# SandraLouise/SVJedi-graph

Hardware: NVIDIA B200
Metric: gaf_alignments_filtered_assigned_per_sec (higher is better)
Workload: dtype u8/int64

## Files before the change

### svjedi-graph_b200/csrc/filter.cu

```cuda
#include <cooperative_groups.h>
#include <cuda_runtime.h>

#include <algorithm>
#include <cstdlib>
#include <map>
#include <mutex>

#include "svjg_internal.h"

namespace cg = cooperative_groups;
using namespace svjg;

namespace {

constexpr int TILE_MIN = 1024;
constexpr int TILE_LINES = 30;
constexpr int LOOKAHEAD = 1024;
constexpr int HEAD = 32;
constexpr int WARPS = 4;
constexpr int THREADS = WARPS * 32;
constexpr int SPARE = 32;

template <int MB_, int TILE_MAX_>
struct Geo {
// ... 606 lines not shown
                }
                const uint32_t idB = node_id(tok_hash(B), B);
                const int sB = strand(B);
                if (err) return;
                link(A, idA, sA, B, idB, sB, false, false);
                if (err) return;
                idA = idB;
                sA = sB;
                have_a = true;
            } else {
                have_a = false;
            }
            A = B;
        }
    }
};

__device__ __forceinline__ uint32_t smem_u32(const void *p) { return (uint32_t)__cvta_generic_to_shared(p); }
__device__ __forceinline__ void mbar_init(uint64_t *bar, uint32_t count) {
    asm volatile("mbarrier.init.shared::cta.b64 [%0], %1;" ::"r"(smem_u32(bar)), "r"(count));
    asm volatile("fence.mbarrier_init.release.cluster;" ::: "memory");
}
__device__ __forceinline__ void mbar_expect_tx(uint64_t *bar, uint32_t bytes) {
    asm volatile("mbarrier.arrive.expect_tx.shared::cta.b64 _, [%0], %1;" ::"r"(smem_u32(bar)), "r"(bytes) : "memory");
}
__device__ __forceinline__ void bulk_g2s(void *dst, const void *src, uint32_t bytes, uint64_t *bar) {
    uint64_t once;
    asm volatile("createpolicy.fractional.L2::evict_first.b64 %0, 1.0;" : "=l"(once));
    asm volatile("cp.async.bulk.shared::cluster.global.mbarrier::complete_tx::bytes.L2::cache_hint [%0], [%1], %2, [%3], %4;" ::"r"(
                     smem_u32(dst)),
                 "l"(src), "r"(bytes), "r"(smem_u32(bar)), "l"(once)
                 : "memory");
}
__device__ __forceinline__ void mbar_wait(uint64_t *bar, uint32_t parity) {
    asm volatile(
        "{\n\t.reg .pred p;\n\t"
        "WAIT_%=:\n\t"
        "mbarrier.try_wait.parity.shared::cta.b64 p, [%0], %1;\n\t"
        "@p bra DONE_%=;\n\t"
        "bra WAIT_%=;\n\t"
        "DONE_%=:\n\t}" ::"r"(smem_u32(bar)),
        "r"(parity)
        : "memory");
}

__device__ __forceinline__ void l2_prefetch(const void *src, uint32_t bytes) {
    asm volatile("cp.async.bulk.prefetch.L2.global [%0], %1;" ::"l"(src), "r"(bytes) : "memory");
}

__device__ __forceinline__ uint32_t lds32(const uint8_t *win, uint32_t a) { return *reinterpret_cast<const uint32_t *>(win + a); }

__device__ __forceinline__ bool has_comma(const uint8_t *win, uint32_t lo, uint32_t hi) {
    const uint32_t a0 = lo & ~3u, a1 = (hi - 1u) & ~3u;
    const uint32_t lom = 0xFFFFFFFFu << (8u * (lo & 3u)), him = 0xFFFFFFFFu >> (8u * (3u - ((hi - 1u) & 3u)));
    uint32_t f = eq_bytes(lds32(win, a0), 0x2C2C2C2Cu) & lom;
    if (a0 == a1) return (f & him) != 0;
    for (uint32_t a = a0 + 4; a < a1; a += 4) f |= eq_bytes(lds32(win, a), 0x2C2C2C2Cu);
    return (f | (eq_bytes(lds32(win, a1), 0x2C2C2C2Cu) & him)) != 0;
}

__device__ __forceinline__ uint32_t warp_incl_scan(uint32_t v, int lane) {
#pragma unroll
    for (int d = 1; d < 32; d <<= 1) {
        uint32_t o = __shfl_up_sync(0xFFFFFFFFu, v, d);
        if (lane >= d) v += o;
    }
    return v;
}

__device__ __forceinline__ uint64_t warp_incl_scan64(uint64_t v, int lane) {
#pragma unroll
    for (int d = 1; d < 32; d <<= 1) {
        uint64_t o = __shfl_up_sync(0xFFFFFFFFu, v, d);
        if (lane >= d) v += o;
    }
    return v;
}

__device__ __forceinline__ uint32_t bm_bits(const uint32_t *bm, uint32_t pos) {
    const uint32_t w = pos >> 5;
    return __funnelshift_r(bm[w], bm[w + 1], pos & 31u);
}
__device__ __forceinline__ uint32_t low_bits(int n) { return __funnelshift_lc(0xFFFFFFFFu, 0u, uint32_t(max(n, 0))); }
__device__ __forceinline__ uint32_t next_tab(const uint32_t *bm, uint32_t pos, uint32_t end) {
    for (uint32_t q = pos; q < end; q += 32) {
        const uint32_t m = bm_bits(bm, q) & low_bits(int(end - q));
        if (m) return q + uint32_t(__ffs(m) - 1);
    }
    return end;
}
__device__ __forceinline__ uint64_t bm64(const uint32_t *bm, uint32_t pos) {
    const uint32_t w = pos >> 5, sh = pos & 31u;
    const uint32_t b0 = bm[w], b1 = bm[w + 1], b2 = bm[w + 2];
    return (uint64_t(__funnelshift_r(b1, b2, sh)) << 32) | __funnelshift_r(b0, b1, sh);
}
__device__ __forceinline__ uint64_t low_bits64(int n) { return (uint64_t(low_bits(n - 32)) << 32) | low_bits(n); }

__device__ __forceinline__ uint32_t dec4(uint32_t w) {
    uint32_t t = w & 0x0F0F0F0Fu;
    t = t * 10u + (t >> 8);
    t &= 0x00FF00FFu;
    return (t * 100u + (t >> 16)) & 0xFFFFu;
}
__device__ __forceinline__ uint32_t clear_low_bytes(uint32_t w, int n) {
    return w & __funnelshift_lc(0u, 0xFFFFFFFFu, uint32_t(max(n, 0)) * 8u);
}
__device__ __forceinline__ bool pnode_find(const DevTables &tb, uint64_t c0, uint64_t c1, uint32_t ka, uint32_t kb,
                                           uint32_t &id, uint32_t &alt_len, uint32_t &roles) {
    uint32_t i = pnode_hash(c0, c1, ka, kb) & tb.pnode_mask;
    for (;;) {
        const uint4 *sp = reinterpret_cast<const uint4 *>(tb.pnodes + i);
        const uint4 lo = __ldg(sp), hi = __ldg(sp + 1);
        if (!hi.z) return false;
        if (lo.x == uint32_t(c0) && lo.y == uint32_t(c0 >> 32) && lo.z == uint32_t(c1) && lo.w == uint32_t(c1 >> 32) &&
            hi.x == ka && hi.y == kb) {
            id = (hi.z & PN_ID_MASK) - 1u;
            roles = hi.z >> 28;
            alt_len = hi.w;
            return true;
        }
        i = (i + 1) & tb.pnode_mask;
    }
}

__device__ __forceinline__ uint32_t link_dirs(uint32_t rolesA, uint32_t sA, uint32_t rolesB, uint32_t sB) {
    const uint32_t fwd = (rolesA >> sA) & (rolesB >> (2u + sB)) & 1u;
    const uint32_t rev = (rolesB >> (sB ^ 1u)) & (rolesA >> (2u + (sA ^ 1u))) & 1u;
    return fwd | (rev << 1);
}

struct SmemBytes {
    const uint8_t *p;
    __device__ __forceinline__ uint32_t u8(uint32_t i) const { return p[i]; }
    __device__ __forceinline__ uint32_t u32(uint32_t al) const { return *reinterpret_cast<const uint32_t *>(p + al); }
};
struct ShardBytes {
    const FilterArgs *a;
    __device__ __forceinline__ uint32_t u8(uint32_t i) const { return i < a->n ? __ldg(a->gaf + i) : 0u; }
    __device__ __forceinline__ uint32_t u32(uint32_t al) const { return gaf_word(*a, al); }
};

template <class B>
__device__ __forceinline__ uint32_t dec9(const B &src, uint32_t hi, uint32_t n) {
    const uint32_t base = hi - 8u, al = base & ~3u, sh = (base & 3u) * 8u;
    const uint32_t r0 = src.u32(al), r1 = src.u32(al + 4), r2 = src.u32(al + 8);
    const int m = 8 - int(min(n, 8u));
    const uint32_t g0 = dec4(clear_low_bytes(__funnelshift_r(r0, r1, sh), m));
    const uint32_t g1 = dec4(clear_low_bytes(__funnelshift_r(r1, r2, sh), m - 4));
    uint32_t v = g0 * 10000u + g1;
    if (n == 9u) v += (src.u8(hi - 9u) - '0') * 100000000u;
    return v;
}

struct Node {
    uint32_t nid = NO_NODE;
    uint32_t nlen = 0;
    uint32_t akey = 0;
    uint32_t roles = 0;
    bool plain = false;
};
template <class B>
__device__ __forceinline__ Node resolve_node(const B &src, const uint32_t *xdb, const DevTables &tb, uint32_t tpos, uint32_t tend) {
    Node n;
    const uint32_t L = tend - tpos;
    const uint32_t Y = bm_bits(xdb, tend - 32u) | low_bits(32 - int(L));
    const uint32_t n2 = uint32_t(__clz(int(Y)));
    const uint32_t n1 = uint32_t(__clz(int(Y << ((n2 + 1u) & 31u))));
    const int clen = int(L) - int(n1 + n2 + 2u);
    if (n2 - 1u <= 8u && n1 - 1u <= 8u && uint32_t(clen) <= 15u) {
        const uint32_t q2 = tend - n2, sep = q2 - 1u, q1 = sep - n1, col = q1 - 1u;
        const uint32_t cs = src.u8(sep);
        bool ok = (cs == '-' || cs == '.') && src.u8(col) == ':';
        ok = ok && !(n1 > 1u && src.u8(q1) == '0') && !(n2 > 1u && src.u8(q2) == '0');
        const uint32_t al = tpos & ~3u, sh = (tpos & 3u) * 8u;
        const uint32_t r0 = src.u32(al), r1 = src.u32(al + 4), r2 = src.u32(al + 8), r3 = src.u32(al + 12), r4 = src.u32(al + 16);
        const uint32_t w0 = __funnelshift_r(r0, r1, sh) & low_bits(8 * clen);
        const uint32_t w1 = __funnelshift_r(r1, r2, sh) & low_bits(8 * clen - 32);
        const uint32_t w2 = __funnelshift_r(r2, r3, sh) & low_bits(8 * clen - 64);
        const uint32_t w3 = (__funnelshift_r(r3, r4, sh) & low_bits(8 * clen - 96)) | (uint32_t(clen) << 24);
        auto has_colon = [](uint32_t w) {
            const uint32_t x = w ^ 0x3A3A3A3Au;
            return (x - 0x01010101u) & ~x & SVJG_H8;
        };
        ok = ok && (has_colon(w0) | has_colon(w1) | has_colon(w2) | has_colon(w3 & 0x00FFFFFFu)) == 0u;
        if (ok) {
            const uint32_t v0 = dec9(src, sep, n1), v1 = dec9(src, tend, n2);
            const uint32_t kind = cs == '.' ? PN_ALT : 0u;
            uint32_t id = NO_NODE, alt_len = PN_NO_LEN;
            const bool found = pnode_find(tb, (uint64_t(w1) << 32) | w0, (uint64_t(w3) << 32) | w2, v0, v1 | kind, id, alt_len, n.roles);
            n.akey = v0 | kind;
            if (!kind) {
                if (v1 >= v0) {
                    n.plain = true;
                    n.nlen = v1 - v0 + 1u;
                    n.nid = found ? id : NO_NODE;
                }
            } else if (found && alt_len != PN_NO_LEN) {
                n.plain = true;
                n.nlen = alt_len;
                n.nid = id;
            }
        }
    }
    return n;
}

__device__ __forceinline__ uint32_t find_node(const uint32_t *nsb, uint32_t lps, uint32_t idx) {
    uint32_t w = lps >> 5, rem = idx;
    uint32_t bits = nsb[w] & ~low_bits(int(lps & 31u));
    for (;;) {
        const uint32_t c = __popc(bits);
        if (rem < c) break;
        rem -= c;
        bits = nsb[++w];
    }
    for (; rem; --rem) bits &= bits - 1;
    return w * 32u + uint32_t(__ffs(bits) - 1);
}
__device__ __forceinline__ uint32_t next_node(const uint32_t *nsb, uint32_t pos, uint32_t end) { return next_tab(nsb, pos, end); }

__device__ __forceinline__ void probe_links(const FilterArgs &a, bool want, uint32_t idl, uint32_t sl, uint32_t idr, uint32_t sr,
                                            uint32_t dirs, bool ok, uint32_t off, uint32_t len, uint32_t lt_mask, uint32_t &n_checks) {
#pragma unroll 1
    for (uint32_t pass = 0; pass < 2; ++pass) {
        const bool act = want && (pass ? dirs == 3u : dirs != 0u);
        if (pass && !__any_sync(0xFFFFFFFFu, act)) break;
        const bool fwd = pass == 0 && (dirs & 1u);
        const uint32_t kl = fwd ? idl : idr, kr = fwd ? idr : idl, ksl = fwd ? sl : sr ^ 1u, ksr = fwd ? sr : sl ^ 1u;
        const uint32_t key_lo = (kr << 1) | ksr, key_hi = (kl << 1) | ksl;
        uint4 sv = make_uint4(0, 0, 0, 0);
        uint32_t i = link_hash((uint64_t(key_hi) << 32) | key_lo);
        bool go = act, match = false;
        while (__any_sync(0xFFFFFFFFu, go)) {
            if (go) {
                i &= a.tb.link_mask;
                sv = __ldg(reinterpret_cast<const uint4 *>(a.tb.links + i));
                match = (sv.w & 1u) && sv.x == key_lo && sv.y == key_hi;
                go = (sv.w & 1u) && !match;
                ++i;
            }
        }
        const bool poisoned = match && (sv.w & 8u);
        const uint32_t cnt = (match && !poisoned) ? sv.w >> 4 : 0u;
        n_checks += cnt;
        const uint32_t mine = ok ? cnt : 0u;
        uint32_t before, total;
        if (__any_sync(0xFFFFFFFFu, mine > 1u)) {
            const uint32_t incl = warp_incl_scan(mine, int(threadIdx.x & 31));
            before = incl - mine;
            total = __shfl_sync(0xFFFFFFFFu, incl, 31);
        } else {
            const uint32_t hb = __ballot_sync(0xFFFFFFFFu, mine != 0u);
            before = __popc(hb & lt_mask);
            total = __popc(hb);
        }
        if (total) {
            unsigned long long base = 0;
            if ((threadIdx.x & 31) == 0) base = atomicAdd(a.stats + 0, (unsigned long long)total);
            base = __shfl_sync(0xFFFFFFFFu, base, 0) + before;
            for (uint32_t k = 0; k < mine; ++k) {
                const uint32_t sv2 = cnt == 1u ? sv.z : __ldg(a.tb.entries + sv.z + k);
                if (sv2 == ENTRY_POISON) {
                    report(a, SVJG_BAD_ENTRY, off);
                    break;
                }
                atomicAdd(a.counts + sv2, 1u);
                if (base + k < a.hit_cap) {
                    __stcs(a.hit_sv2 + base + k, sv2);
                    if (a.hit_off64) __stcs(reinterpret_cast<unsigned long long *>(a.hit_off64) + base + k, (unsigned long long)(a.base + off));
                    else __stcs(a.hit_off + base + k, off);
                    __stcs(a.hit_len + base + k, len);
                }
            }
        }
        if (poisoned) report(a, SVJG_BAD_ENTRY, off);
    }
}

constexpr int SLAB_N = 256;

template <class B>
__device__ __noinline__ bool long_line(const FilterArgs &a, const B src, const uint32_t *nsb, const uint32_t *xdb, uint4 *slab,
                                       uint32_t slab_cap, int lane, uint32_t cnt, uint32_t lps, uint32_t lpe, int64_t lts,
                                       int64_t ltail, uint32_t off, uint32_t len) {
    if (cnt > slab_cap) return false;
    const uint32_t lt_mask = (1u << lane) - 1u;
    uint32_t n_checks = 0;
    uint64_t total = 0;
    bool bad = false;
    uint32_t from = lps;
    for (uint32_t c0 = 0; c0 < cnt; c0 += 32) {
        const bool act = c0 + uint32_t(lane) < cnt;
        Node n;
        uint32_t tpos = lpe, plus = 0;
        if (act) tpos = find_node(nsb, from, uint32_t(lane));
        uint32_t nxt = __shfl_down_sync(0xFFFFFFFFu, tpos, 1);
        if (lane == 31 && act && c0 + 32u < cnt) nxt = next_node(nsb, tpos + 1u, lpe);
        if (act) {
            const uint32_t tend = c0 + uint32_t(lane) + 1u < cnt ? nxt - 1u : lpe;
            plus = src.u8(tpos - 1u) == '>';
            n = resolve_node(src, xdb, a.tb, tpos, tend);
            __stcg(slab + c0 + lane, make_uint4(n.nid, n.nlen, n.akey, plus | (n.roles << 1)));
        }
        bad |= __any_sync(0xFFFFFFFFu, act && !n.plain);
        total += __shfl_sync(0xFFFFFFFFu, warp_incl_scan64(n.nlen, lane), 31);
        from = __shfl_sync(0xFFFFFFFFu, nxt, 31);
    }
    __syncwarp();
    if (bad) return false;
    bool clash = false;
    for (uint32_t c0 = 0; c0 < cnt; c0 += 32) {
        const uint32_t t = c0 + uint32_t(lane);
        const uint32_t mine = t < cnt ? __ldcg(&slab[t].z) : 0u;
        const uint32_t upto = min(c0 + 32u, cnt);
        for (uint32_t j = 0; j < upto; ++j) clash |= j < t && t < cnt && __ldcg(&slab[j].z) == mine;
    }
    if (__any_sync(0xFFFFFFFFu, clash)) return false;
    uint64_t before = 0;
    for (uint32_t c0 = 0; c0 < cnt; c0 += 32) {
        const uint32_t t = c0 + uint32_t(lane);
        const bool act = t < cnt;
        const uint4 me = act ? __ldcg(slab + t) : make_uint4(NO_NODE, 0, 0, 0);
        const uint4 lf = act && t ? __ldcg(slab + t - 1) : make_uint4(NO_NODE, 0, 0, 0);
        const uint64_t incl = warp_incl_scan64(me.y, lane);
        const uint64_t pre = before + incl - me.y;
        const bool ok = (int64_t(pre) - lts >= a.d_over) && (int64_t(total - pre) - ltail >= a.d_over);
        const uint32_t dirs = link_dirs(lf.w >> 1, lf.w & 1u, me.w >> 1, me.w & 1u);
        const bool want = act && t && lf.x != NO_NODE && me.x != NO_NODE && dirs && (ok || (a.flags & FLAG_EXACT_CHECKS));
        probe_links(a, want, lf.x, lf.w & 1u, me.x, me.w & 1u, dirs, ok, off, len, lt_mask, n_checks);
        before += __shfl_sync(0xFFFFFFFFu, incl, 31);
    }
    n_checks = __reduce_add_sync(0xFFFFFFFFu, n_checks);
    if (lane == 0 && n_checks) atomicAdd(a.stats + 3, (unsigned long long)n_checks);
    return true;
}

template <class G>
__global__ void __launch_bounds__(THREADS, G::MB) scan_kernel(const __grid_constant__ FilterArgs a) {
    extern __shared__ __align__(128) uint8_t smem_all[];
    __shared__ __align__(8) uint64_t mbars[WARPS];
    __shared__ uint32_t next_tile[WARPS];

    const int lane = threadIdx.x & 31, warp = threadIdx.x >> 5;
    const uint32_t lt_mask = (1u << lane) - 1u;
    uint8_t *win = smem_all + warp * G::WARP_SMEM;
    uint16_t *nl = reinterpret_cast<uint16_t *>(win + G::OFF_NL);
    uint32_t *tabb = reinterpret_cast<uint32_t *>(win + G::OFF_TAB);
    uint32_t *xdb = reinterpret_cast<uint32_t *>(win + G::OFF_XD);
    uint32_t *nsb = reinterpret_cast<uint32_t *>(win + G::OFF_NS);
    uint8_t *tko = win + G::OFF_TKO;
    uint2 *lrec = reinterpret_cast<uint2 *>(win + G::OFF_LREC);
    uint64_t *mbar = &mbars[warp];
    const SmemBytes src{win};

    if (lane == 0) mbar_init(mbar, 1);
    for (int i = lane; i < G::BMWORDS; i += 32) tabb[i] = 0, xdb[i] = 0, nsb[i] = 0;
    for (int i = G::WIN + lane; i < G::WIN + SPARE; i += 32) win[i] = 0;
    __syncwarp();
    uint32_t phase = 0;
    uint32_t u_rec = 0, u_multi = 0, n_checks = 0;
    const uint32_t one = a.one;
    const uint32_t n_workers = gridDim.x * WARPS;

    cudaGridDependencySynchronize();
    cudaTriggerProgrammaticLaunchCompletion();
    const uint32_t tile_bytes = a.sc.cnt[4];
    const uint32_t n_tiles = uint32_t((a.n + tile_bytes - 1) / tile_bytes);
    const uint32_t win_bytes = HEAD + tile_bytes + LOOKAHEAD, n_pairs = win_bytes / 32u;

    for (uint32_t tile = blockIdx.x * WARPS + warp; tile < n_tiles; tile = next_tile[warp], __syncwarp()) {
        const uint64_t tile_start = uint64_t(tile) * tile_bytes;
        const uint64_t g0 = tile_start ? tile_start - HEAD : 0;
        const uint32_t dst0 = tile_start ? 0 : HEAD;
        uint64_t g1 = tile_start + tile_bytes + LOOKAHEAD;
        if (g1 > a.n) g1 = a.n;
        const bool at_eof = (g1 == a.n);
        const uint32_t nbytes = uint32_t(g1 - g0);
        const uint32_t bulk = nbytes & ~15u;
        const uint32_t valid_end = dst0 + nbytes;
        const uint32_t wbase = uint32_t(tile_start) - HEAD;

        if (lane == 0) {
            if (bulk) {
                asm volatile("fence.proxy.async.shared::cta;" ::: "memory");
                mbar_expect_tx(mbar, bulk);
                bulk_g2s(win + dst0, a.gaf + g0, bulk, mbar);
            }
            const uint32_t next = n_workers + atomicAdd(a.sc.cnt + 6, 1u);
            next_tile[warp] = next;
            const uint64_t nx = uint64_t(next) * tile_bytes;
            if (nx + tile_bytes + LOOKAHEAD <= a.n) l2_prefetch(a.gaf + nx - HEAD, win_bytes);
        }
        if (bulk != nbytes || dst0 || valid_end < win_bytes) {
            for (uint32_t i = bulk + lane; i < nbytes; i += 32) win[dst0 + i] = __ldg(a.gaf + g0 + i);
            if (dst0) win[lane] = (lane == HEAD - 1 && a.skip == 0u) ? '\n' : 0;
            for (uint32_t i = valid_end + lane; i < win_bytes; i += 32) win[i] = 0;
        }
        if (bulk) {
            mbar_wait(mbar, phase);
            phase ^= 1;
        }
        __syncwarp();

        const uint32_t own_end = min(HEAD + tile_bytes, valid_end);
        uint32_t n_nl = 0, n_own = 0;
        for (uint32_t c0 = 0; c0 < n_pairs; c0 += 32) {
            const uint32_t c = c0 + uint32_t(lane);
            const uint32_t p0 = c * 32u;
            uint32_t m = 0;
            if (c < n_pairs) {
                const uint4 v0 = *reinterpret_cast<const uint4 *>(win + p0);
                const uint4 v1 = *reinterpret_cast<const uint4 *>(win + p0 + 16);
                m = mask32(v0, v1, IsNewline{one});
                tabb[c] = mask32(v0, v1, IsTab{one});
                xdb[c] = mask32(v0, v1, IsNonDigit{one});
                const uint32_t d = mask32(v0, v1, IsDelim{one});
                const uint32_t left = c ? uint32_t(is_delim(win[p0 - 1u])) : 0u;
                nsb[c] = ((d << 1) | left) & ~d;
                if (c == 0) m &= 0x80000000u;
            }
            if (__any_sync(0xFFFFFFFFu, (m & (m - 1u)) != 0u)) {
                const uint32_t cnt = __popc(m), incl = warp_incl_scan(cnt, lane);
                uint32_t idx = n_nl + incl - cnt, own = 0;
                for (uint32_t mm = m; mm; mm &= mm - 1) {
                    const uint32_t pos = p0 + uint32_t(__ffs(mm) - 1);
                    if (idx < uint32_t(G::NLCAP)) nl[idx] = uint16_t(pos);
                    own += pos + 1u < own_end;
                    ++idx;
                }
                n_nl += __shfl_sync(0xFFFFFFFFu, incl, 31);
                n_own += __reduce_add_sync(0xFFFFFFFFu, own);
            } else {
                const uint32_t pos = p0 + uint32_t(__ffs(m)) - 1u;
                const uint32_t b = __ballot_sync(0xFFFFFFFFu, m != 0u);
                const uint32_t bo = __ballot_sync(0xFFFFFFFFu, m != 0u && pos + 1u < own_end);
                const uint32_t idx = n_nl + __popc(b & lt_mask);
                if (m != 0u && idx < uint32_t(G::NLCAP)) nl[idx] = uint16_t(pos);
                n_nl += __popc(b);
                n_own += __popc(bo);
            }
            if ((c0 + 32u) * 32u >= own_end && __any_sync(0xFFFFFFFFu, (m & ~low_bits(int(own_end) - 1 - int(p0))) != 0)) break;
        }
        __syncwarp();
        if (a.flags & FLAG_STOP_AFTER_SCAN) continue;

        if (n_nl > uint32_t(G::NLCAP)) {
            if (lane == 0) report(a, SVJG_BAD_SHORTLINE, tile_start);
            __syncwarp();
            continue;
        }
        u_rec += n_own;
        for (uint32_t k0 = 0; k0 < n_own; k0 += 32) {
            const uint32_t k = k0 + lane;
            uint32_t want = 0;
            bool exact = false;
            uint32_t s = 0, e = 0, ps = 0, pe = 0;
            uint32_t c6 = 0, c7 = 0, c8 = 0, c9 = 0;
            bool has_nl = false;
            if (k < n_own) {
                s = uint32_t(nl[k]) + 1u;
                if (k + 1 < n_nl) {
                    e = nl[k + 1];
                    has_nl = true;
                } else if (at_eof) {
                    e = valid_end;
                } else {
                    exact = true;
                }
                if (!exact) {
                    bool plain = e > s && !py_space(win[e - 1]);
                    uint32_t t1;
                    {
                        const uint64_t t64 = bm64(tabb, s) & low_bits64(int(e - s));
                        t1 = t64 ? s + uint32_t(__ffsll((long long)t64)) - 1u : next_tab(tabb, min(s + 64u, e), e);
                    }
                    plain &= t1 < e;
                    const uint32_t n2 = t1 + 1u;
                    const uint32_t tw = bm_bits(tabb, n2);
                    const uint32_t xa = bm_bits(xdb, n2) & ~tw;
                    plain &= xa != 0;
                    const uint32_t l2 = uint32_t(__ffs(xa)) - 1u;
                    const uint32_t ta = tw & low_bits(int(l2));
                    plain &= __popc(ta) == 3 && (ta >> ((l2 - 1u) & 31u)) == 1u && (ta & ((ta >> 1) | 1u)) == 0;
                    const uint32_t n5 = n2 + l2;
                    ps = (l2 < 31u && ((tw >> (l2 + 1u)) & 1u)) ? n5 + 2u : next_tab(tabb, min(n5, e), e) + 1u;
                    uint32_t ntok = 0;
                    pe = e;
                    for (uint32_t q = ps; q < e; q += 32) {
                        const uint32_t tb = bm_bits(tabb, q) & low_bits(int(e - q));
                        const uint32_t nb = bm_bits(nsb, q);
                        if (tb) {
                            const uint32_t r = uint32_t(__ffs(tb)) - 1u;
                            pe = q + r;
                            ntok += __popc(nb & low_bits(int(r)));
                            break;
                        }
                        ntok += __popc(nb);
                    }
                    plain &= pe < e && pe > ps;
                    const uint32_t n7 = min(pe + 1u, e);
                    uint64_t tt = bm64(tabb, n7);
                    const uint64_t xt = bm64(xdb, n7) & ~tt;
                    plain &= xt != 0;
                    const uint32_t l7 = uint32_t(__ffsll((long long)xt)) - 1u;
                    tt &= low_bits64(int(l7));
                    const uint32_t ntab = uint32_t(__popcll(tt));
                    const bool last_is_tab = l7 != 0 && ((tt >> ((l7 - 1u) & 63u)) & 1ull) != 0;
                    plain &= (ntab == 6 && last_is_tab) || (ntab == 5 && !last_is_tab && n7 + l7 == e);
                    plain &= (tt & ((tt >> 1) | 1ull)) == 0;
                    c6 = pe;
                    c7 = n7 + uint32_t(__ffsll((long long)tt)) - 1u;
                    tt &= tt - 1;
                    c8 = n7 + uint32_t(__ffsll((long long)tt)) - 1u;
                    tt &= tt - 1;
                    c9 = n7 + uint32_t(__ffsll((long long)tt)) - 1u;
                    tt &= tt - 1;
                    const uint32_t p10 = n7 + uint32_t(__ffsll((long long)tt)) - 1u;
                    plain = plain && win[p10 + 1] != '0';
                    if (!plain) {
                        exact = true;
                    } else if (!is_delim(win[ps])) {
                        exact = has_comma(win, ps, pe);
                    } else if (ntok >= 2) {
                        if (a.flags & FLAG_FORCE_GENERAL) exact = true;
                        else want = ntok;
                    }
                }
            }
            __syncwarp();
            int32_t ts = 0, tail = 0;
            if (want) {
                const uint32_t n_tlen = c7 - c6 - 1u, n_ts = c8 - c7 - 1u, n_te = c9 - c8 - 1u;
                if (max(n_tlen, max(n_ts, n_te)) <= 9u) {
                    ts = int32_t(dec9(src, c8, n_ts));
                    tail = int32_t(dec9(src, c7, n_tlen)) - int32_t(dec9(src, c9, n_te)) - 1;
                    lrec[lane] = make_uint2(s | ((e - s + (has_nl ? 1u : 0u)) << 16), ps | (pe << 16));
                } else {
                    exact = true;
                    want = 0;
                }
            }
            __syncwarp();
            uint32_t pend = want > 32u ? 0u : want;
            while (__any_sync(0xFFFFFFFFu, pend != 0)) {
                const uint32_t incl = warp_incl_scan(pend, lane);
                const bool take = pend != 0 && incl <= 32u;
                const uint32_t takeb = __ballot_sync(0xFFFFFFFFu, take);
                const uint32_t ntk = __shfl_sync(0xFFFFFFFFu, incl, 31 - __clz(takeb));
                const uint32_t first = incl - pend;
                const uint32_t startmask = __reduce_or_sync(0xFFFFFFFFu, take ? (1u << first) : 0u);
                if (take) tko[__popc(takeb & lt_mask)] = uint8_t(lane);
                __syncwarp();
                const bool is_tok = uint32_t(lane) < ntk;
                uint32_t own_l = 0, idx = 0;
                if (is_tok) {
                    const uint32_t below = startmask & (0xFFFFFFFFu >> (31 - lane));
                    own_l = tko[__popc(below) - 1];
                    idx = uint32_t(lane) - uint32_t(31 - __clz(below));
                }
                const uint2 lr = lrec[own_l];
                const uint32_t lpath = lr.y;
                const uint32_t lcnt = __shfl_sync(0xFFFFFFFFu, pend, own_l);
                uint32_t tpos = 0;
                if (is_tok) tpos = find_node(nsb, lpath & 0xFFFFu, idx);
                const uint32_t nxt = __shfl_down_sync(0xFFFFFFFFu, tpos, 1);
                Node nd;
                uint32_t plus = 0;
                if (is_tok) {
                    plus = win[tpos - 1u] == '>';
                    nd = resolve_node(src, xdb, a.tb, tpos, idx + 1u < lcnt ? nxt - 1u : lpath >> 16);
                }
                const uint32_t nid = nd.nid, nlen = nd.nlen, akey = nd.akey;
                const uint32_t lfirst = uint32_t(lane) - idx;
                const uint32_t line_lanes = low_bits(int(lcnt)) << lfirst;
                const uint32_t twins = __match_any_sync(0xFFFFFFFFu, akey) & line_lanes;
                bool clash = (twins & ~(1u << lane)) != 0;
                uint64_t lsum = nlen;
#pragma unroll
                for (int d = 1; d < 32; d <<= 1) {
                    const uint64_t o = __shfl_up_sync(0xFFFFFFFFu, lsum, d);
                    if (uint32_t(d) <= idx) lsum += o;
                }
                uint64_t pre_l = lsum - nlen, pre_r = pre_l;
                uint32_t splus = plus, sl = __shfl_up_sync(0xFFFFFFFFu, plus, 1);
                if (__any_sync(0xFFFFFFFFu, is_tok && clash)) {
                    const int twin0 = is_tok ? __ffs(twins) - 1 : lane;
                    const uint32_t f_nid = __shfl_sync(0xFFFFFFFFu, nid, twin0);
                    const uint64_t f_sum = __shfl_sync(0xFFFFFFFFu, lsum, twin0);
                    const uint32_t f_len = __shfl_sync(0xFFFFFFFFu, nlen, twin0);
                    splus = __shfl_sync(0xFFFFFFFFu, plus, twin0);
                    sl = __shfl_up_sync(0xFFFFFFFFu, splus, 1);
                    pre_l = __shfl_up_sync(0xFFFFFFFFu, f_sum, 1);
                    pre_r = f_sum - f_len;
                    clash = clash && !(nid != NO_NODE && f_nid == nid);
                }
                const uint32_t bad = __reduce_or_sync(0xFFFFFFFFu, (is_tok && (!nd.plain || clash)) ? (1u << own_l) : 0u);
                const uint64_t total = __shfl_sync(0xFFFFFFFFu, lsum, is_tok ? lfirst + lcnt - 1u : 0u);
                const uint32_t idl = __shfl_up_sync(0xFFFFFFFFu, nid, 1);
                const int64_t lts = __shfl_sync(0xFFFFFFFFu, ts, own_l), ltail = __shfl_sync(0xFFFFFFFFu, tail, own_l);
                const uint32_t loff = wbase + (lr.x & 0xFFFFu), llen = lr.x >> 16;
                const bool ok = (int64_t(pre_l) - lts >= a.d_over) && (int64_t(total - pre_r) - ltail >= a.d_over);
                const uint32_t dirs = link_dirs(__shfl_up_sync(0xFFFFFFFFu, nd.roles, 1), sl, nd.roles, splus);
                const bool look = is_tok && idx >= 1 && !((bad >> own_l) & 1u) && idl != NO_NODE && nid != NO_NODE && dirs &&
                                  (ok || (a.flags & FLAG_EXACT_CHECKS));
                probe_links(a, look, idl, sl, nid, splus, dirs, ok, loff, llen, lt_mask, n_checks);
                if (take) {
                    if ((bad >> lane) & 1u) exact = true;
                    pend = 0;
                }
                u_multi += __popc(takeb & ~bad);
                __syncwarp();
            }
            for (uint32_t longb = __ballot_sync(0xFFFFFFFFu, want > 32u); longb; longb &= longb - 1) {
                const int L = __ffs(longb) - 1;
                const uint2 lr = lrec[L];
                const bool done = long_line(a, src, nsb, xdb, a.sc.slab + size_t(blockIdx.x * WARPS + warp) * SLAB_N, SLAB_N, lane,
                                            __shfl_sync(0xFFFFFFFFu, want, L), lr.y & 0xFFFFu, lr.y >> 16,
                                            __shfl_sync(0xFFFFFFFFu, ts, L), __shfl_sync(0xFFFFFFFFu, tail, L),
                                            wbase + (lr.x & 0xFFFFu), lr.x >> 16);
                if (!done && lane == L) exact = true;
                u_multi += done;
            }
            const uint32_t xb = __ballot_sync(0xFFFFFFFFu, exact);
            if (xb) {
                uint32_t xbase = 0;
                if (lane == 0) xbase = atomicAdd(a.sc.cnt + 2, uint32_t(__popc(xb)));
                xbase = __shfl_sync(0xFFFFFFFFu, xbase, 0);
                if (exact) {
                    const uint32_t idx = xbase + __popc(xb & lt_mask);
                    if (idx < a.sc.cap_exact) a.sc.exact[idx] = wbase + s;
                    else report(a, SVJG_BAD_SHORTLINE, wbase + s);
                }
            }
        }
        __syncwarp();
    }
    n_checks = __reduce_add_sync(0xFFFFFFFFu, n_checks);
    if (lane == 0) {
        if (u_rec) atomicAdd(a.stats + 1, (unsigned long long)u_rec);
        if (u_multi) atomicAdd(a.stats + 2, (unsigned long long)u_multi);
        if (n_checks) atomicAdd(a.stats + 3, (unsigned long long)n_checks);
    }
}

__device__ __noinline__ bool giant_line(const FilterArgs &a, uint32_t ps, uint32_t pe, uint32_t ntok, int64_t ts, int64_t tail,
                                        uint32_t off, uint32_t len, int lane, Local &loc) {
    if (ps < 64u) return false;
    const uint32_t w0 = (ps >> 5) - 1u, nw = (pe >> 5) - w0 + 4u;
    const uint32_t bm16 = (nw + 3u) / 4u;
    const uint32_t need = 2u * bm16 + ntok;
    uint32_t base = 0;
    if (lane == 0) base = atomicAdd(a.sc.cnt + 5, need);
    base = __shfl_sync(0xFFFFFFFFu, base, 0);
    if (uint64_t(base) + need > a.sc.cap_pool) return false;
    uint32_t *nsb = reinterpret_cast<uint32_t *>(a.sc.pool + base), *xdb = reinterpret_cast<uint32_t *>(a.sc.pool + base + bm16);
    for (uint32_t w = uint32_t(lane); w < nw; w += 32) {
        const uint64_t pos = uint64_t(w0 + w) * 32u;
        uint32_t d = 0, x = 0;
        if (pos + 32 <= a.n) {
            const uint4 v0 = __ldg(reinterpret_cast<const uint4 *>(a.gaf + pos)), v1 = __ldg(reinterpret_cast<const uint4 *>(a.gaf + pos + 16));
            d = mask16(v0, IsDelim{1u}) | (mask16(v1, IsDelim{1u}) << 16);
            x = mask16(v0, IsNonDigit{1u}) | (mask16(v1, IsNonDigit{1u}) << 16);
        } else {
            for (uint32_t k = 0; k < 32; ++k) {
                const uint32_t c = pos + k < a.n ? uint32_t(__ldg(a.gaf + pos + k)) : 0u;
                d |= uint32_t(is_delim(c)) << k;
                x |= uint32_t(c - '0' > 9u) << k;
            }
        }
        const uint32_t left = uint32_t(is_delim(__ldg(a.gaf + pos - 1)));
        __stcg(nsb + w, ((d << 1) | left) & ~d);
        __stcg(xdb + w, x);
    }
    __syncwarp();
    return long_line(a, ShardBytes{&a}, nsb - w0, xdb - w0, a.sc.pool + base + 2u * bm16, ntok, lane, ntok, ps, pe, ts, tail, off, len);
}

__global__ void __launch_bounds__(FLAT_THREADS) exact_kernel(const __grid_constant__ FilterArgs a) {
    cudaGridDependencySynchronize();
    cudaTriggerProgrammaticLaunchCompletion();
    const uint32_t n = min(a.sc.cnt[2], a.sc.cap_exact);
    if (n == 0) return;
    Local loc;
    const uint32_t n_warps = gridDim.x * (FLAT_THREADS / 32);
    const bool per_warp = n <= 4u * n_warps;
    const uint32_t me = per_warp ? (blockIdx.x * FLAT_THREADS + threadIdx.x) >> 5 : blockIdx.x * FLAT_THREADS + threadIdx.x;
    const uint32_t stride = per_warp ? n_warps : gridDim.x * FLAT_THREADS;
    const uint32_t part = per_warp ? (threadIdx.x & 31u) : 0u, parts = per_warp ? 32u : 1u;
    if (blockIdx.x == 0 && threadIdx.x == 0 && n) atomicAdd(a.stats + 7, (unsigned long long)n);
    for (uint32_t i = me; i < n; i += stride) {
        const uint32_t off = a.sc.exact[i];
        uint64_t e = off;
        if (per_warp) e = coop_find(a, off, a.n, EqByte{0x0A0A0A0Au});
        else
            while (e < a.n && __ldg(a.gaf + e) != '\n') ++e;
        const uint32_t len = uint32_t(e - off) + (e < a.n ? 1u : 0u);
        Rec<GmemSrc> rec(a, GmemSrc{a.gaf}, off, len, loc);
        rec.coop = per_warp;
        const uint32_t ntok = rec.parse_fields(uint64_t(off), e);
        if (!rec.err && ntok >= 2) {
            if (ntok != COMMA_PATH && part == 0) loc.n_multi++;
            const bool fast = per_warp && ntok != COMMA_PATH && !(a.flags & FLAG_FORCE_GENERAL) && e < 0xFFFFFFFFull &&
                              giant_line(a, uint32_t(rec.ps), uint32_t(rec.pe), ntok, rec.ts, rec.tlen - rec.te - 1, off, len,
                                         int(threadIdx.x & 31u), loc);
            if (!fast) rec.general(part, parts);
        }
        if (rec.err) report(a, rec.err, off);
    }
    add_stats(a, loc);
}

constexpr int PROBE_THREADS = 1024, PROBE_BYTES = 64 << 10;

__global__ void __launch_bounds__(PROBE_THREADS) probe_kernel(const __grid_constant__ FilterArgs a) {
    cudaTriggerProgrammaticLaunchCompletion();
    __shared__ uint32_t total;
    if (threadIdx.x == 0) total = 0;
    if (threadIdx.x < 16 && threadIdx.x != 4) a.sc.cnt[threadIdx.x] = 0;
    __syncthreads();
    const uint64_t span = a.n < uint64_t(PROBE_BYTES) ? a.n : uint64_t(PROBE_BYTES);
    const uint32_t n16 = uint32_t(span / 16);
    const uint4 *p = reinterpret_cast<const uint4 *>(a.gaf);
    uint32_t cnt = 0;
    for (uint32_t i = threadIdx.x; i < n16; i += PROBE_THREADS) {
        const uint4 v = __ldg(p + i);
        cnt += __popc(eq_bytes(v.x, 0x0A0A0A0Au)) + __popc(eq_bytes(v.y, 0x0A0A0A0Au)) + __popc(eq_bytes(v.z, 0x0A0A0A0Au)) +
               __popc(eq_bytes(v.w, 0x0A0A0A0Au));
    }
    cnt = __reduce_add_sync(0xFFFFFFFFu, cnt);
    if ((threadIdx.x & 31) == 0 && cnt) atomicAdd(&total, cnt);
    __syncthreads();
    if (threadIdx.x == 0) {
        const uint32_t tile_max = a.tile_max;
        uint32_t tile = tile_max;
        if (total) {
            const uint64_t want = uint64_t(n16) * 16ull * a.tile_lines / total;
            tile = uint32_t(want < uint64_t(tile_max) ? want : uint64_t(tile_max)) & ~31u;
        }
        if (const uint32_t forced = (a.flags >> 16)) tile = forced & ~31u;
        if (total) {
            const uint64_t s15 = uint64_t(n16) * 24ull / total;
            const uint32_t slack = uint32_t(s15 < 512 ? s15 : 512);
            tile = min(tile, tile_max);
            const uint32_t steps = (HEAD + tile + slack) / 1024u;
            if (steps >= 2) tile = (steps * 1024u - HEAD - slack) & ~31u;
        }
        a.sc.cnt[4] = max(uint32_t(TILE_MIN), min(tile, tile_max));
    }
}

__global__ void reset_kernel(uint32_t *counts, uint64_t n, unsigned long long *stats) {
    uint64_t i = blockIdx.x * uint64_t(blockDim.x) + threadIdx.x;
    uint64_t stride = uint64_t(gridDim.x) * blockDim.x;
    for (uint64_t k = i; k < n; k += stride) counts[k] = 0;
    if (i < 8) stats[i] = (i == 5) ? ~0ull : 0ull;
}

template <typename... P, typename... A>
cudaError_t launch_pdl(void (*kernel)(P...), unsigned grid, unsigned block, size_t smem, cudaStream_t st, A &&...args) {
    cudaLaunchAttribute attr[1];
    attr[0].id = cudaLaunchAttributeProgrammaticStreamSerialization;
    attr[0].val.programmaticStreamSerializationAllowed = 1;
    cudaLaunchConfig_t cfg = {};
    cfg.gridDim = dim3(grid);
    cfg.blockDim = dim3(block);
    cfg.dynamicSmemBytes = smem;
    cfg.stream = st;
    cfg.attrs = attr;
    cfg.numAttrs = 1;
    return cudaLaunchKernelEx(&cfg, kernel, static_cast<A &&>(args)...);
}

struct DevCfg {
    int sms = 0;
    int grid_cap = 0;
    int min_blocks = 0;
    uint32_t tile_max = 0, tile_lines = 0;
    uint32_t smem = 0;
    cudaEvent_t ev0 = nullptr, ev1 = nullptr;
    bool timed = false;
};
std::mutex g_cfg_mu;
std::map<int, DevCfg> g_cfg;
bool g_profile = false;

struct Knobs {
    int tile_bytes = 0, tile_lines = 0, scan_blocks = 0, scan_only = 0, pool_units = 0;
};
Knobs g_knobs;

// ... 164 lines not shown
```

Measured before the change: 8.061 billion.

## Prefetch next tile's window during final node-table lookups of current tile

Splits node resolution into key parsing from the shared-memory window and a separate hash-table lookup. On the last batch of a tile, once every remaining read of the window is done, lane 0 starts the bulk async copy of the next tile's window before the table lookups run. This is meant to hide the global-to-shared copy latency behind those lookups. It also packs two per-lane counters into one register. It adds a shared flag and a condition on when the window is dead, which risks a race if any later code still reads the window.

```diff
diff --git a/svjedi-graph_b200/csrc/filter.cu b/svjedi-graph_b200/csrc/filter.cu
--- a/svjedi-graph_b200/csrc/filter.cu
+++ b/svjedi-graph_b200/csrc/filter.cu
@@ -782,6 +782,11 @@
     return v;
 }
 
+struct NodeKey {
+    uint32_t w0 = 0, w1 = 0, w2 = 0, w3 = 0;
+    uint32_t ka = 0, kb = 0;
+    bool ok = false;
+};
 struct Node {
     uint32_t nid = NO_NODE;
     uint32_t nlen = 0;
@@ -790,8 +795,8 @@
     bool plain = false;
 };
 template <class B>
-__device__ __forceinline__ Node resolve_node(const B &src, const uint32_t *xdb, const DevTables &tb, uint32_t tpos, uint32_t tend) {
-    Node n;
+__device__ __forceinline__ NodeKey node_key(const B &src, const uint32_t *xdb, uint32_t tpos, uint32_t tend) {
+    NodeKey k;
     const uint32_t L = tend - tpos;
     const uint32_t Y = bm_bits(xdb, tend - 32u) | low_bits(32 - int(L));
     const uint32_t n2 = uint32_t(__clz(int(Y)));
@@ -814,22 +819,31 @@
         };
         ok = ok && (has_colon(w0) | has_colon(w1) | has_colon(w2) | has_colon(w3 & 0x00FFFFFFu)) == 0u;
         if (ok) {
-            const uint32_t v0 = dec9(src, sep, n1), v1 = dec9(src, tend, n2);
-            const uint32_t kind = cs == '.' ? PN_ALT : 0u;
-            uint32_t id = NO_NODE, alt_len = PN_NO_LEN;
-            const bool found = pnode_find(tb, (uint64_t(w1) << 32) | w0, (uint64_t(w3) << 32) | w2, v0, v1 | kind, id, alt_len, n.roles);
-            n.akey = v0 | kind;
-            if (!kind) {
-                if (v1 >= v0) {
-                    n.plain = true;
-                    n.nlen = v1 - v0 + 1u;
-                    n.nid = found ? id : NO_NODE;
-                }
-            } else if (found && alt_len != PN_NO_LEN) {
+            k.w0 = w0, k.w1 = w1, k.w2 = w2, k.w3 = w3;
+            k.ka = dec9(src, sep, n1);
+            k.kb = dec9(src, tend, n2) | (cs == '.' ? PN_ALT : 0u);
+            k.ok = true;
+        }
+    }
+    return k;
+}
+__device__ __forceinline__ Node node_find(const DevTables &tb, const NodeKey &k) {
+    Node n;
+    if (k.ok) {
+        const uint32_t v0 = k.ka, kind = k.kb & PN_ALT, v1 = k.kb & ~PN_ALT;
+        uint32_t id = NO_NODE, alt_len = PN_NO_LEN;
+        const bool found = pnode_find(tb, (uint64_t(k.w1) << 32) | k.w0, (uint64_t(k.w3) << 32) | k.w2, k.ka, k.kb, id, alt_len, n.roles);
+        n.akey = v0 | kind;
+        if (!kind) {
+            if (v1 >= v0) {
                 n.plain = true;
-                n.nlen = alt_len;
-                n.nid = id;
-            }
+                n.nlen = v1 - v0 + 1u;
+                n.nid = found ? id : NO_NODE;
+            }
+        } else if (found && alt_len != PN_NO_LEN) {
+            n.plain = true;
+            n.nlen = alt_len;
+            n.nid = id;
         }
     }
     return n;
@@ -929,7 +943,7 @@
         if (act) {
             const uint32_t tend = c0 + uint32_t(lane) + 1u < cnt ? nxt - 1u : lpe;
             plus = src.u8(tpos - 1u) == '>';
-            n = resolve_node(src, xdb, a.tb, tpos, tend);
+            n = node_find(a.tb, node_key(src, xdb, tpos, tend));
             __stcg(slab + c0 + lane, make_uint4(n.nid, n.nlen, n.akey, plus | (n.roles << 1)));
         }
         bad |= __any_sync(0xFFFFFFFFu, act && !n.plain);
@@ -970,6 +984,7 @@
     extern __shared__ __align__(128) uint8_t smem_all[];
     __shared__ __align__(8) uint64_t mbars[WARPS];
     __shared__ uint32_t next_tile[WARPS];
+    __shared__ uint32_t next_copied[WARPS];
 
     const int lane = threadIdx.x & 31, warp = threadIdx.x >> 5;
     const uint32_t lt_mask = (1u << lane) - 1u;
@@ -983,12 +998,12 @@
     uint64_t *mbar = &mbars[warp];
     const SmemBytes src{win};
 
-    if (lane == 0) mbar_init(mbar, 1);
+    if (lane == 0) mbar_init(mbar, 1), next_copied[warp] = 0;
     for (int i = lane; i < G::BMWORDS; i += 32) tabb[i] = 0, xdb[i] = 0, nsb[i] = 0;
     for (int i = G::WIN + lane; i < G::WIN + SPARE; i += 32) win[i] = 0;
     __syncwarp();
     uint32_t phase = 0;
-    uint32_t u_rec = 0, u_multi = 0, n_checks = 0;
+    uint32_t u_lines = 0, n_checks = 0;
     const uint32_t one = a.one;
     const uint32_t n_workers = gridDim.x * WARPS;
 
@@ -996,7 +1011,7 @@
     cudaTriggerProgrammaticLaunchCompletion();
     const uint32_t tile_bytes = a.sc.cnt[4];
     const uint32_t n_tiles = uint32_t((a.n + tile_bytes - 1) / tile_bytes);
-    const uint32_t win_bytes = HEAD + tile_bytes + LOOKAHEAD, n_pairs = win_bytes / 32u;
+    const uint32_t win_bytes = HEAD + tile_bytes + LOOKAHEAD;
 
     for (uint32_t tile = blockIdx.x * WARPS + warp; tile < n_tiles; tile = next_tile[warp], __syncwarp()) {
         const uint64_t tile_start = uint64_t(tile) * tile_bytes;
@@ -1011,7 +1026,9 @@
         const uint32_t wbase = uint32_t(tile_start) - HEAD;
 
         if (lane == 0) {
-            if (bulk) {
+            if (next_copied[warp]) {
+                next_copied[warp] = 0;
+            } else if (bulk) {
                 asm volatile("fence.proxy.async.shared::cta;" ::: "memory");
                 mbar_expect_tx(mbar, bulk);
                 bulk_g2s(win + dst0, a.gaf + g0, bulk, mbar);
@@ -1034,6 +1051,7 @@
 
         const uint32_t own_end = min(HEAD + tile_bytes, valid_end);
         uint32_t n_nl = 0, n_own = 0;
+        const uint32_t n_pairs = win_bytes / 32u;
         for (uint32_t c0 = 0; c0 < n_pairs; c0 += 32) {
             const uint32_t c = c0 + uint32_t(lane);
             const uint32_t p0 = c * 32u;
@@ -1079,7 +1097,7 @@
             __syncwarp();
             continue;
         }
-        u_rec += n_own;
+        u_lines += lane == 0 ? n_own : 0u;
         for (uint32_t k0 = 0; k0 < n_own; k0 += 32) {
             const uint32_t k = k0 + lane;
             uint32_t want = 0;
@@ -1194,12 +1212,26 @@
                 uint32_t tpos = 0;
                 if (is_tok) tpos = find_node(nsb, lpath & 0xFFFFu, idx);
                 const uint32_t nxt = __shfl_down_sync(0xFFFFFFFFu, tpos, 1);
-                Node nd;
+                NodeKey key;
                 uint32_t plus = 0;
                 if (is_tok) {
                     plus = win[tpos - 1u] == '>';
-                    nd = resolve_node(src, xdb, a.tb, tpos, idx + 1u < lcnt ? nxt - 1u : lpath >> 16);
-                }
+                    key = node_key(src, xdb, tpos, idx + 1u < lcnt ? nxt - 1u : lpath >> 16);
+                }
+                if (k0 + 32u >= n_own && __ballot_sync(0xFFFFFFFFu, pend != 0u) == takeb && !__any_sync(0xFFFFFFFFu, want > 32u)) {
+                    __syncwarp();
+                    if (lane == 0) {
+                        const uint64_t nx = uint64_t(next_tile[warp]) * tile_bytes;
+                        if (nx + tile_bytes + LOOKAHEAD <= a.n) {
+                            asm volatile("fence.proxy.async.shared::cta;" ::: "memory");
+                            mbar_expect_tx(mbar, win_bytes);
+                            bulk_g2s(win, a.gaf + nx - HEAD, win_bytes, mbar);
+                            next_copied[warp] = 1;
+                        }
+                    }
+                }
+                Node nd;
+                if (is_tok) nd = node_find(a.tb, key);
                 const uint32_t nid = nd.nid, nlen = nd.nlen, akey = nd.akey;
                 const uint32_t lfirst = uint32_t(lane) - idx;
                 const uint32_t line_lanes = low_bits(int(lcnt)) << lfirst;
@@ -1238,7 +1270,7 @@
                     if ((bad >> lane) & 1u) exact = true;
                     pend = 0;
                 }
-                u_multi += __popc(takeb & ~bad);
+                u_lines += lane == 1 ? __popc(takeb & ~bad) : 0u;
                 __syncwarp();
             }
             for (uint32_t longb = __ballot_sync(0xFFFFFFFFu, want > 32u); longb; longb &= longb - 1) {
@@ -1249,7 +1281,7 @@
                                             __shfl_sync(0xFFFFFFFFu, ts, L), __shfl_sync(0xFFFFFFFFu, tail, L),
                                             wbase + (lr.x & 0xFFFFu), lr.x >> 16);
                 if (!done && lane == L) exact = true;
-                u_multi += done;
+                u_lines += lane == 1 ? uint32_t(done) : 0u;
             }
             const uint32_t xb = __ballot_sync(0xFFFFFFFFu, exact);
             if (xb) {
@@ -1266,6 +1298,7 @@
         __syncwarp();
     }
     n_checks = __reduce_add_sync(0xFFFFFFFFu, n_checks);
+    const uint32_t u_rec = __shfl_sync(0xFFFFFFFFu, u_lines, 0), u_multi = __shfl_sync(0xFFFFFFFFu, u_lines, 1);
     if (lane == 0) {
         if (u_rec) atomicAdd(a.stats + 1, (unsigned long long)u_rec);
         if (u_multi) atomicAdd(a.stats + 2, (unsigned long long)u_multi);
```

Result: no change. 8.011 billion, median of 6 (-0.6%).

## Compute delimiter bitmaps only over path columns, cooperatively across the warp

Applied to the files above, without the earlier changes.

The scan phase no longer builds the node-start delimiter bitmap for every 32-byte chunk of the window. After each lane has located its line's path column, the warp builds a load-balanced list of only the words covering those path spans, computes the node-start mask for them, and accumulates per-line token counts via shared atomics. This removes delimiter-mask work on bytes outside path fields and replaces the per-lane serial token loop, at the cost of an extra warp scan, a binary-search shuffle per word and shared-memory atomics. A profiling script for the scan phase is also added.

```diff
diff --git a/profiles/scan_phase_a.py b/profiles/scan_phase_a.py
--- /dev/null
+++ b/profiles/scan_phase_a.py
@@ -0,0 +1,67 @@
+#!/usr/bin/env python3
+import argparse
+import ctypes as C
+import json
+import os
+import subprocess
+import sys
+
+ROOT = os.path.dirname(os.path.dirname(os.path.abspath(__file__)))
+sys.path[:0] = [ROOT, os.path.join(ROOT, "svjedi-graph_b200")]
+
+
+def main():
+    ap = argparse.ArgumentParser()
+    ap.add_argument("--workload", default="C2", choices=("C2", "C3", "C4", "C5"))
+    ap.add_argument("--scale", type=float, default=None)
+    ap.add_argument("--catalogue", default="scaled", choices=("scaled", "full"))
+    ap.add_argument("--iters", type=int, default=50)
+    ap.add_argument("--warmup", type=int, default=5)
+    args = ap.parse_args()
+
+    import torch
+
+    import bench
+    from svjg import alnfilter, capi
+
+    g, _vcf, gaf, gfa_text, _scale, _gen_s = bench.workload(args, 0)
+    tables = alnfilter.Tables.from_memory(g.edges_json(), gfa_text).to_device(0)
+    raw = gaf.encode() if isinstance(gaf, str) else gaf
+    d_gaf = torch.frombuffer(bytearray(raw), dtype=torch.uint8).cuda()
+    filt = alnfilter.DeviceFilter(tables, hit_cap=1024)
+    filt.run(d_gaf)
+    filt = alnfilter.DeviceFilter(tables, hit_cap=filt.read_stats()["n_hits"] + 1024)
+    stream = torch.cuda.current_stream()
+    sp = C.c_void_p(stream.cuda_stream)
+    lib = capi.lib
+
+    def timed(n):
+        tot, ms = 0.0, C.c_float()
+        for _ in range(n):
+            capi.check(lib.svjg_filter_reset(filt.counts.data_ptr(), tables.num_sv, filt.stats.data_ptr(), sp))
+            capi.check(lib.svjg_filter_device(tables._h, d_gaf.data_ptr(), d_gaf.numel(), 0, 100, filt.counts.data_ptr(),
+                                              filt.hit_sv2.data_ptr(), filt.hit_off.data_ptr(), filt.hit_len.data_ptr(),
+                                              filt.hit_cap, filt.stats.data_ptr(), sp))
+            capi.check(lib.svjg_filter_scan_ms(C.byref(ms)))
+            tot += ms.value
+        return tot / n
+
+    out = {"workload": args.workload, "catalogue": args.catalogue, "bytes": d_gaf.numel(), "iters": args.iters}
+    capi.check(lib.svjg_filter_profile(1))
+    try:
+        for key, only in (("scan_ms", 0), ("phase_a_ms", 1)):
+            capi.check(lib.svjg_filter_tune(capi.TUNE_SCAN_ONLY, only))
+            timed(args.warmup)
+            out[key] = timed(args.iters)
+    finally:
+        capi.check(lib.svjg_filter_tune(capi.TUNE_SCAN_ONLY, 0))
+        capi.check(lib.svjg_filter_profile(0))
+    smi = subprocess.run(["nvidia-smi", "--query-gpu=name,power.limit,clocks.sm,clocks.max.sm", "--format=csv,noheader", "-i", "0"],
+                         capture_output=True, text=True)
+    out["gpu"] = smi.stdout.strip()
+    print(json.dumps(out))
+    tables.close()
+
+
+if __name__ == "__main__":
+    main()
diff --git a/svjedi-graph_b200/csrc/filter.cu b/svjedi-graph_b200/csrc/filter.cu
--- a/svjedi-graph_b200/csrc/filter.cu
+++ b/svjedi-graph_b200/csrc/filter.cu
@@ -1044,9 +1044,6 @@
                 m = mask32(v0, v1, IsNewline{one});
                 tabb[c] = mask32(v0, v1, IsTab{one});
                 xdb[c] = mask32(v0, v1, IsNonDigit{one});
-                const uint32_t d = mask32(v0, v1, IsDelim{one});
-                const uint32_t left = c ? uint32_t(is_delim(win[p0 - 1u])) : 0u;
-                nsb[c] = ((d << 1) | left) & ~d;
                 if (c == 0) m &= 0x80000000u;
             }
             if (__any_sync(0xFFFFFFFFu, (m & (m - 1u)) != 0u)) {
@@ -1084,6 +1081,7 @@
             const uint32_t k = k0 + lane;
             uint32_t want = 0;
             bool exact = false;
+            bool nodes = false;
             uint32_t s = 0, e = 0, ps = 0, pe = 0;
             uint32_t c6 = 0, c7 = 0, c8 = 0, c9 = 0;
             bool has_nl = false;
@@ -1114,19 +1112,7 @@
                     plain &= __popc(ta) == 3 && (ta >> ((l2 - 1u) & 31u)) == 1u && (ta & ((ta >> 1) | 1u)) == 0;
                     const uint32_t n5 = n2 + l2;
                     ps = (l2 < 31u && ((tw >> (l2 + 1u)) & 1u)) ? n5 + 2u : next_tab(tabb, min(n5, e), e) + 1u;
-                    uint32_t ntok = 0;
-                    pe = e;
-                    for (uint32_t q = ps; q < e; q += 32) {
-                        const uint32_t tb = bm_bits(tabb, q) & low_bits(int(e - q));
-                        const uint32_t nb = bm_bits(nsb, q);
-                        if (tb) {
-                            const uint32_t r = uint32_t(__ffs(tb)) - 1u;
-                            pe = q + r;
-                            ntok += __popc(nb & low_bits(int(r)));
-                            break;
-                        }
-                        ntok += __popc(nb);
-                    }
+                    pe = next_tab(tabb, ps, e);
                     plain &= pe < e && pe > ps;
                     const uint32_t n7 = min(pe + 1u, e);
                     uint64_t tt = bm64(tabb, n7);
@@ -1151,13 +1137,48 @@
                         exact = true;
                     } else if (!is_delim(win[ps])) {
                         exact = has_comma(win, ps, pe);
-                    } else if (ntok >= 2) {
-                        if (a.flags & FLAG_FORCE_GENERAL) exact = true;
-                        else want = ntok;
+                    } else {
+                        nodes = true;
                     }
                 }
             }
             __syncwarp();
+            {
+                const uint32_t w0 = ps >> 5, nw = nodes ? ((pe - 1u) >> 5) - w0 + 1u : 0u;
+                const uint32_t incl = warp_incl_scan(nw, lane);
+                const uint32_t n_words = __shfl_sync(0xFFFFFFFFu, incl, 31);
+                const uint32_t wadd = w0 + nw - incl;
+                lrec[lane].x = 0u;
+                __syncwarp();
+#pragma unroll 1
+                for (uint32_t j0 = 0; j0 < n_words; j0 += 32) {
+                    const uint32_t j = j0 + uint32_t(lane);
+                    uint32_t L = 0;
+#pragma unroll
+                    for (uint32_t st = 16; st; st >>= 1)
+                        if (__shfl_sync(0xFFFFFFFFu, incl, L + st - 1u) <= j) L += st;
+                    const uint32_t c = j + __shfl_sync(0xFFFFFFFFu, wadd, L);
+                    const int lps = __shfl_sync(0xFFFFFFFFu, int(ps), L), lpe = __shfl_sync(0xFFFFFFFFu, int(pe), L);
+                    if (j < n_words) {
+                        const uint32_t p0 = c * 32u;
+                        const uint4 v0 = *reinterpret_cast<const uint4 *>(win + p0);
+                        const uint4 v1 = *reinterpret_cast<const uint4 *>(win + p0 + 16);
+                        const uint32_t d = mask32(v0, v1, IsDelim{one});
+                        const uint32_t ns = ((d << 1) | uint32_t(is_delim(win[p0 - 1u]))) & ~d;
+                        nsb[c] = ns;
+                        const uint32_t in_path = ~low_bits(lps - int(p0)) & low_bits(lpe - int(p0));
+                        atomicAdd(&lrec[L].x, uint32_t(__popc(ns & in_path)));
+                    }
+                }
+                __syncwarp();
+            }
+            if (nodes) {
+                const uint32_t ntok = lrec[lane].x;
+                if (ntok >= 2) {
+                    if (a.flags & FLAG_FORCE_GENERAL) exact = true;
+                    else want = ntok;
+                }
+            }
             int32_t ts = 0, tail = 0;
             if (want) {
                 const uint32_t n_tlen = c7 - c6 - 1u, n_ts = c8 - c7 - 1u, n_te = c9 - c8 - 1u;
```

After: 8.029 billion before, 8.072 billion after, median of 6. Within noise of the previous version (+0.5%).
